# chenglou/ai-font-renderer

Measured on AMD Instinct MI355X. Metric: glyphs/sec training (batch fwd+bwd+step), higher is better.
Workload: dtype bf16; 1 GPU; C3: 32x32 glyph MLP 32->1024->1024->1024, char+font embedding, batch 8192/GPU (BASELINE configs[2]; per-GPU shard of configs[3]); per_gpu_batch=8192, global_batch=8192, parallelism=single, params=2137152

## Files before the change

ai-font-renderer_amd/csrc/afr_api.hip:

```cpp
#include "afr_common.h"
#include "../../include/afr.h"
static_assert(AFR_LOSS_MSE == LOSS_MSE && AFR_LOSS_BCE == LOSS_BCE, "afr.h and afr_common.h name the same loss kinds");

#include <cmath>
#include <cstdarg>
#include <cstdio>
#include <cstring>
#include <map>
#include <string>
#include <utility>
#include <vector>

static thread_local char g_err[512] = "";
static int fail(int code, const char* fmt, ...) {
    va_list ap;
    va_start(ap, fmt);
    vsnprintf(g_err, sizeof g_err, fmt, ap);
    va_end(ap);
    return code;
}
#define HIPCHK(expr)                                                                          \
    do {                                                                                      \
        hipError_t e_ = (expr);                                                               \
        if (e_ != hipSuccess) return fail(AFR_EHIP, "%s: %s", #expr, hipGetErrorString(e_)); \
// ... 2405 lines not shown
    if (tokens < 1) return fail(AFR_EINVAL, "afr_op_pixel_add_ln: tokens = %d must be >= 1", tokens);
    DevGuard dg(device_of(h));
    HIPCHK(afr_launch_pixel_add_ln(act_dtype, hin, h, pos, add, g, b, n, rows, tokens, d, eps, (hipStream_t)stream));
    return AFR_OK;
}
extern "C" int afr_op_pixel_attn(int act_dtype, const void* q, const void* kv, void* o, int64_t rows, int tokens, int d, int heads, int C,
                                 void* stream) {
    if (int rc = pixel_op_shape("afr_op_pixel_attn", act_dtype, rows, d)) return rc;
    if (int rc = pixel_op_attn_shape("afr_op_pixel_attn", tokens, d, heads, C)) return rc;
    if (!q || !kv || !o) return fail(AFR_EINVAL, "afr_op_pixel_attn: null argument");
    DevGuard dg(device_of(o));
    HIPCHK(afr_launch_pixel_attn(act_dtype, q, kv, o, rows, tokens, d, heads, C, (hipStream_t)stream));
    return AFR_OK;
}
extern "C" int afr_op_pixel_attn_bwd(int act_dtype, const void* dO, const void* q, const void* kv, void* dq, float* dkv_part, int B, int tokens,
                                     int d, int heads, int C, void* stream) {
    if (int rc = pixel_op_shape("afr_op_pixel_attn_bwd", act_dtype, B, d)) return rc;
    if (int rc = pixel_op_attn_shape("afr_op_pixel_attn_bwd", tokens, d, heads, C)) return rc;
    if (!dO || !q || !kv || !dq || !dkv_part) return fail(AFR_EINVAL, "afr_op_pixel_attn_bwd: null argument");
    const int chunk = afr_pixel_attn_chunk(tokens);
    if ((long long)B * ((tokens + chunk - 1) / chunk) >= (1ll << 31)) return fail(AFR_EUNSUPPORTED, "afr_op_pixel_attn_bwd: B * chunks must stay below 2^31");
    DevGuard dg(device_of(dq));
    HIPCHK(afr_launch_pixel_attn_bwd(act_dtype, dO, q, kv, dq, dkv_part, B, tokens, d, C, (hipStream_t)stream));
    return AFR_OK;
}
extern "C" int afr_op_pixel_head(int act_dtype, int loss_kind, const float* hin, float* h, const void* add, const float* g, const float* b,
                                 const float* w_out, const float* b_out, float* u, float* y, int64_t rows, int d, float eps, void* stream) {
    if (int rc = pixel_op_shape("afr_op_pixel_head", act_dtype, rows, d)) return rc;
    if (loss_kind != AFR_LOSS_MSE && loss_kind != AFR_LOSS_BCE) return fail(AFR_EINVAL, "afr_op_pixel_head: loss kind must be AFR_LOSS_MSE (0) or AFR_LOSS_BCE (1), got %d", loss_kind);
    if (!hin || !h || !add || !g || !b || !w_out || !b_out) return fail(AFR_EINVAL, "afr_op_pixel_head: null argument");
    DevGuard dg(device_of(h));
    HIPCHK(afr_launch_pixel_head(act_dtype, hin, h, add, g, b, w_out, b_out, u, y, rows, d, eps, (hipStream_t)stream, loss_kind));
    return AFR_OK;
}
extern "C" int afr_op_pixel_head_bwd(int act_dtype, const float* du, const float* hf, const float* g, const float* b, const float* w_out, float* dh,
                                     void* dhT, float* part, int64_t rows, int d, float eps, void* stream) {
    if (int rc = pixel_op_shape("afr_op_pixel_head_bwd", act_dtype, rows, d)) return rc;
    if (!du || !hf || !g || !b || !w_out || !dh || !part) return fail(AFR_EINVAL, "afr_op_pixel_head_bwd: null argument");
    DevGuard dg(device_of(dh));
    HIPCHK(afr_launch_pixel_head_bwd(act_dtype, du, hf, g, b, w_out, dh, dhT, part, rows, d, eps, (hipStream_t)stream));
    return AFR_OK;
}
extern "C" int afr_op_pixel_ln_bwd(int act_dtype, const void* dy, const float* hin, const float* g, float* dh, void* dhT, float* part, int64_t rows,
                                   int d, float eps, void* stream) {
    if (int rc = pixel_op_shape("afr_op_pixel_ln_bwd", act_dtype, rows, d)) return rc;
    if (!dy || !hin || !g || !dh || !part) return fail(AFR_EINVAL, "afr_op_pixel_ln_bwd: null argument");
    DevGuard dg(device_of(dh));
    HIPCHK(afr_launch_pixel_ln_bwd(act_dtype, dy, hin, g, dh, dhT, part, rows, d, eps, (hipStream_t)stream));
    return AFR_OK;
}

static int sheet_op_args(const char* what, int act_dtype, const afr_sheet_params* P, const int64_t* x, int ldx, int B, int L, int max_length,
                         int vocab, const afr_sheet_dropout* drop) {
    if (act_dtype != AFR_F32 && act_dtype != AFR_BF16) return fail(AFR_EINVAL, "%s: act_dtype must be AFR_F32 or AFR_BF16, got %d", what, act_dtype);
    if (B < 1) return fail(AFR_EINVAL, "%s: B = %d must be >= 1", what, B);
    if (L < 1) return fail(AFR_EINVAL, "%s: L = %d must be >= 1", what, L);
    if (max_length < 1 || vocab < 1) return fail(AFR_EINVAL, "%s: max_length = %d, vocab = %d must be >= 1", what, max_length, vocab);
    if (L > max_length) return fail(AFR_EINVAL, "%s: L = %d exceeds max_length = %d", what, L, max_length);
    if (L > 120) return fail(AFR_EUNSUPPORTED, "%s: L = %d exceeds 120 (a string's state must fit one compute unit's LDS)", what, L);
    if (ldx < L) return fail(AFR_EINVAL, "%s: ldx = %d is below L = %d", what, ldx, L);
    if ((long long)max_length * 32 >= (1ll << 31) || (long long)vocab * 32 >= (1ll << 31)) return fail(AFR_EUNSUPPORTED, "%s: a table must stay below 2^31 floats", what);
    if (!P || !x) return fail(AFR_EINVAL, "%s: null argument", what);
    if (!P->pos || !P->emb || !P->w_in || !P->b_in || !P->w_o || !P->b_o || !P->ln_g || !P->ln_b || !P->w1 || !P->b1)
        return fail(AFR_EINVAL, "%s: null parameter pointer", what);
    if (drop) {
        const float ps[3] = {drop->p_embed, drop->p_attn, drop->p_fc};
        for (float pr : ps)
            if (!(pr >= 0.f && pr < 1.f)) return fail(AFR_EINVAL, "%s: dropout rate %g outside [0, 1)", what, (double)pr);
    }
    return AFR_OK;
}
static SheetParams sheet_op_params(const afr_sheet_params* P) {
    SheetParams sp;
    sp.pos = P->pos; sp.emb = P->emb; sp.w_in = P->w_in; sp.b_in = P->b_in; sp.w_o = P->w_o; sp.b_o = P->b_o;
    sp.ln_g = P->ln_g; sp.ln_b = P->ln_b; sp.w1 = P->w1; sp.b1 = P->b1;
    return sp;
}
static SheetDrop sheet_op_drop(const afr_sheet_dropout* drop, float* save) {
    if (!drop) return sheet_drop(0, 0, 0, 0.f, 0.f, 0.f, 0, save);
    return sheet_drop(drop->seed, drop->step, drop->rank, drop->p_embed, drop->p_attn, drop->p_fc, 1, save);
}
extern "C" size_t afr_sheet_save_floats(int B, int L) {
    return B > 0 && L > 0 ? (size_t)B * (size_t)L * AFR_SHEET_SAVE_PER_POS : 0;
}
extern "C" int afr_op_sheet_fwd(int act_dtype, const afr_sheet_params* params, const int64_t* x, int ldx, int B, int L, int max_length, int vocab,
                                float ln_eps, const afr_sheet_dropout* drop, void* z, float* save, uint32_t* err, void* stream) {
    if (int rc = sheet_op_args("afr_op_sheet_fwd", act_dtype, params, x, ldx, B, L, max_length, vocab, drop)) return rc;
    if (!z) return fail(AFR_EINVAL, "afr_op_sheet_fwd: null argument");
    DevGuard dg(device_of(z));
    SheetDims d{L, max_length, 32, 4, 64, vocab};
    HIPCHK(afr_launch_sheet_fwd(act_dtype, d, sheet_op_params(params), sheet_op_drop(drop, save), x, ldx, B, z, ln_eps, err, (hipStream_t)stream));
    return AFR_OK;
}
extern "C" int afr_op_sheet_bwd(int act_dtype, const afr_sheet_params* params, const int64_t* x, int ldx, int B, int L, int max_length, int vocab,
                                float ln_eps, const afr_sheet_dropout* drop, const void* dz, const float* save, float* slabs,
                                const afr_sheet_slab_layout* lay, void* stream) {
    const char* what = "afr_op_sheet_bwd";
    if (int rc = sheet_op_args(what, act_dtype, params, x, ldx, B, L, max_length, vocab, drop)) return rc;
    if (!dz || !slabs || !lay) return fail(AFR_EINVAL, "%s: null argument", what);
    if (lay->total < 4 || (lay->total & 3)) return fail(AFR_EINVAL, "%s: total = %d must be a positive multiple of 4 (a block zeroes its slab 16 bytes at a time)", what, lay->total);
    if ((uintptr_t)slabs & 15) return fail(AFR_EINVAL, "%s: slabs must be 16-byte aligned", what);
    const long long off[10] = {lay->pos, lay->emb, lay->w_in, lay->b_in, lay->w_o, lay->b_o, lay->ln_g, lay->ln_b, lay->w1, lay->b1};
    const long long len[10] = {(long long)max_length * 32, (long long)vocab * 32, 96 * 32, 96, 32 * 32, 32, 32, 32, 64 * 32, 64};
    for (int i = 0; i < 10; ++i) {
        if (off[i] < 0 || off[i] + len[i] > lay->total) return fail(AFR_EINVAL, "%s: tensor %d (offset %lld, %lld floats) lies outside total = %d", what, i, off[i], len[i], lay->total);
        for (int j = 0; j < i; ++j)
            if (off[i] < off[j] + len[j] && off[j] < off[i] + len[i]) return fail(AFR_EINVAL, "%s: tensors %d and %d overlap", what, j, i);
    }
    DevGuard dg(device_of(slabs));
    SheetDims d{L, max_length, 32, 4, 64, vocab};
    SheetSlabOff so{lay->pos, lay->emb, lay->w_in, lay->b_in, lay->w_o, lay->b_o, lay->ln_g, lay->ln_b, lay->w1, lay->b1, lay->total};
    HIPCHK(afr_launch_sheet_bwd(act_dtype, d, sheet_op_params(params), sheet_op_drop(drop, const_cast<float*>(save)), x, ldx, B, dz, ln_eps, slabs, so,
                                (hipStream_t)stream));
    return AFR_OK;
}

constexpr size_t GLYPH_OP_LDS_MAX = 160 * 1024;
static int glyph_op_shape(const char* what, int act_dtype, int B, int E, int vocab, int n_fonts) {
    if (act_dtype != AFR_F32 && act_dtype != AFR_BF16) return fail(AFR_EINVAL, "%s: act_dtype must be AFR_F32 or AFR_BF16, got %d", what, act_dtype);
    if (B < 1) return fail(AFR_EINVAL, "%s: B = %d must be >= 1", what, B);
    if (vocab < 1 || n_fonts < 0) return fail(AFR_EINVAL, "%s: vocab = %d, n_fonts = %d", what, vocab, n_fonts);
    if (E < 8 || E % 8) return fail(AFR_EUNSUPPORTED, "%s: E = %d must be a positive multiple of 8", what, E);
    if ((long long)(vocab + (long long)n_fonts) * E >= (1ll << 31)) return fail(AFR_EUNSUPPORTED, "%s: a table must stay below 2^31 floats", what);
    return AFR_OK;
}
static int glyph_op_n1(const char* what, int N1) {
    if (N1 < 8 || N1 % 8) return fail(AFR_EUNSUPPORTED, "%s: N1 = %d must be a positive multiple of 8", what, N1);
    return AFR_OK;
}
static int glyph_op_fold(const char* what, int E, int vocab, int n_fonts) {
    const long long K0 = (long long)E + ((long long)vocab + n_fonts + 7) / 8 * 8;
    if (K0 > 512 || E > 128) return fail(AFR_EUNSUPPORTED, "%s: K0 = %lld, E = %d: the folded first layer takes K0 <= 512 and E <= 128", what, K0, E);
    return AFR_OK;
}
static int glyph_op_lds(const char* what, size_t lds) {
    if (lds > GLYPH_OP_LDS_MAX) return fail(AFR_EUNSUPPORTED, "%s: %zu bytes of dynamic LDS requested, above 160 KiB", what, lds);
    return AFR_OK;
}
extern "C" int afr_op_glyph_embed(int act_dtype, const float* emb, const float* femb, const int64_t* x, const int64_t* font, int B, int E, int vocab,
                                  int n_fonts, void* out, uint32_t* err, void* stream) {
    const char* what = "afr_op_glyph_embed";
    if (int rc = glyph_op_shape(what, act_dtype, B, E, vocab, n_fonts)) return rc;
    if (!emb || !x || !out || !err || (n_fonts > 0 && !femb)) return fail(AFR_EINVAL, "%s: null argument", what);
    DevGuard dg(device_of(out));
    HIPCHK(afr_launch_glyph_embed(act_dtype, emb, femb, x, font, B, E, vocab, n_fonts, out, err, (hipStream_t)stream));
    return AFR_OK;
}
extern "C" int afr_op_glyph_combo(const float* emb, const float* femb, const float* W1, const float* b1, const int64_t* x, const int64_t* font, int B,
                                  int E, int N1, int vocab, int n_fonts, void* h1c, int ld1, void* h0c, int32_t* cidx, void* w1t, uint32_t* err,
                                  void* stream) {
    const char* what = "afr_op_glyph_combo";
    if (int rc = glyph_op_shape(what, AFR_BF16, B, E, vocab, n_fonts)) return rc;
    if (int rc = glyph_op_n1(what, N1)) return rc;
    const size_t lds = (size_t)(256 * (E + 1) + 2 * 4 * E) * sizeof(float);
    if (lds > 48 * 1024) return fail(AFR_EUNSUPPORTED, "%s: E = %d needs %zu bytes of staging, above the kernel's 48 KiB (E <= 40)", what, E, lds);
    if (ld1 < N1) return fail(AFR_EINVAL, "%s: ld1 = %d is below N1 = %d", what, ld1, N1);
    if ((long long)vocab * (n_fonts > 0 ? n_fonts : 1) * (long long)ld1 >= (1ll << 31)) return fail(AFR_EUNSUPPORTED, "%s: the combination table must stay below 2^31 elements", what);
    if (!emb || !W1 || !b1 || !x || !h1c || !h0c || !cidx || !err || (n_fonts > 0 && !femb)) return fail(AFR_EINVAL, "%s: null argument", what);
    if ((uintptr_t)W1 & 15) return fail(AFR_EINVAL, "%s: W1 must be 16-byte aligned", what);
    DevGuard dg(device_of(h1c));
    HIPCHK(afr_launch_glyph_combo(emb, femb, W1, b1, x, font, B, E, N1, vocab, n_fonts, nullptr, h1c, ld1, h0c, cidx, err, (hipStream_t)stream, w1t));
    return AFR_OK;
}
extern "C" int afr_op_glyph_l1_bwd(const float* slabs, int nslabs, long long slab_stride, const float* W1, int N1, int E, int vocab, int n_fonts,
                                   float* dw1, float* dtab_part, void* stream) {
    const char* what = "afr_op_glyph_l1_bwd";
    if (int rc = glyph_op_shape(what, AFR_F32, 1, E, vocab, n_fonts)) return rc;
    if (int rc = glyph_op_n1(what, N1)) return rc;
    if (int rc = glyph_op_fold(what, E, vocab, n_fonts)) return rc;
    const int K0 = afr_glyph_k0(E, vocab, n_fonts);
    if (nslabs < 1) return fail(AFR_EINVAL, "%s: nslabs = %d must be >= 1", what, nslabs);
    if (slab_stride % 4 || (nslabs > 1 && slab_stride < (long long)N1 * K0))
        return fail(AFR_EINVAL, "%s: slab_stride = %lld must be a multiple of 4 and at least N1 * K0 = %lld", what, slab_stride, (long long)N1 * K0);
    if (!slabs || !W1 || !dw1 || !dtab_part) return fail(AFR_EINVAL, "%s: null argument", what);
    if ((uintptr_t)slabs & 15) return fail(AFR_EINVAL, "%s: slabs must be 16-byte aligned", what);
    const int G = std::max(1, std::min(1024 / (8 * K0 / 4), 8));
    if (int rc = glyph_op_lds(what, ((size_t)8 * (K0 + E) + (size_t)(G - 1) * 8 * K0) * sizeof(float))) return rc;
    DevGuard dg(device_of(dw1));
    HIPCHK(afr_launch_glyph_l1_bwd(slabs, nslabs, slab_stride, W1, N1, E, vocab, n_fonts, dw1, dtab_part, (hipStream_t)stream));
    return AFR_OK;
}
extern "C" int afr_op_glyph_l1_bwd_fused(const void* d1, const void* h0, int ldh, const int32_t* h0_rowmap, const void* W1T, const int64_t* x,
                                         const int64_t* font, int B, int N1, int vocab, int n_fonts, float* slabs, void* stream) {
    const char* what = "afr_op_glyph_l1_bwd_fused";
    if (int rc = glyph_op_shape(what, AFR_BF16, B, 32, vocab, n_fonts)) return rc;
    if (int rc = glyph_op_n1(what, N1)) return rc;
    if (!afr_glyph_l1_bwd_fused_eligible(AFR_BF16, 32, N1, vocab, n_fonts))
        return fail(AFR_EUNSUPPORTED, "%s: N1 = %d, vocab + n_fonts = %d: the fused backward takes N1 a multiple of 128 in 256 .. 1024 and at most 144 table rows (E = 32)",
                    what, N1, vocab + n_fonts);
    if (ldh < 32 || ldh % 8) return fail(AFR_EINVAL, "%s: ldh = %d must be a multiple of 8, at least 32", what, ldh);
    if ((long long)B * N1 * 2 >= (1ll << 31) || (!h0_rowmap && (long long)B * ldh * 2 >= (1ll << 31)))
        return fail(AFR_EUNSUPPORTED, "%s: d1 and h0 must stay below 2 GiB", what);
    if (!d1 || !h0 || !W1T || !x || !slabs) return fail(AFR_EINVAL, "%s: null argument", what);
    if (((uintptr_t)d1 & 15) || ((uintptr_t)h0 & 15) || ((uintptr_t)W1T & 15) || ((uintptr_t)slabs & 15))
        return fail(AFR_EINVAL, "%s: d1, h0, W1T and slabs must be 16-byte aligned", what);
    if (int rc = glyph_op_lds(what, (size_t)(N1 / afr_glyph_l1_bwd_fused_split(B, N1) / 128 + 1) * 16384 + 2 * 64 * sizeof(int))) return rc;
    DevGuard dg(device_of(slabs));
    HIPCHK(afr_launch_glyph_l1_bwd_fused(d1, N1, h0, ldh, W1T, x, font, B, N1, vocab, n_fonts, slabs, (hipStream_t)stream, h0_rowmap, nullptr));
    return AFR_OK;
}
extern "C" int afr_op_glyph_embed_bwd(int act_dtype, const void* d, const int64_t* x, const int64_t* font, int B, int E, int vocab, int n_fonts,
                                      float* slabs, void* stream) {
    const char* what = "afr_op_glyph_embed_bwd";
    if (int rc = glyph_op_shape(what, act_dtype, B, E, vocab, n_fonts)) return rc;
    if (int rc = glyph_op_lds(what, afr_glyph_embed_bwd_lds_bytes(E, vocab, n_fonts))) return rc;
    if (!d || !x || !slabs) return fail(AFR_EINVAL, "%s: null argument", what);
    DevGuard dg(device_of(slabs));
    HIPCHK(afr_launch_glyph_embed_bwd(act_dtype, d, x, font, B, E, vocab, n_fonts, slabs, (hipStream_t)stream));
    return AFR_OK;
}

extern "C" int afr_op_glyph_l1_fwd(int act_dtype, const float* emb, const float* femb, const float* W1, const float* b1, const int64_t* x,
                                   const int64_t* font, int B, int E, int N1, int vocab, int n_fonts, float* table, void* h0p, void* h1, void* w1t,
                                   uint32_t* err, void* stream) {
    const char* what = "afr_op_glyph_l1_fwd";
    if (int rc = glyph_op_shape(what, act_dtype, B, E, vocab, n_fonts)) return rc;
    if (int rc = glyph_op_n1(what, N1)) return rc;
    if (int rc = glyph_op_fold(what, E, vocab, n_fonts)) return rc;
    if ((long long)B * std::max(N1, afr_glyph_k0(E, vocab, n_fonts)) >= (1ll << 31) || (long long)(vocab + n_fonts) * N1 >= (1ll << 31))
        return fail(AFR_EUNSUPPORTED, "%s: h1, h0' and the table must stay below 2^31 elements", what);
    if (!emb || !W1 || !b1 || !x || !table || !h0p || !h1 || !err || (n_fonts > 0 && !femb)) return fail(AFR_EINVAL, "%s: null argument", what);
    if (((uintptr_t)emb & 15) || (n_fonts > 0 && ((uintptr_t)femb & 15)) ||((uintptr_t)W1 & 15) || ((uintptr_t)b1 & 15) || ((uintptr_t)table & 15) ||
        ((uintptr_t)h0p & 15) || ((uintptr_t)h1 & 15))
        return fail(AFR_EINVAL, "%s: emb, femb, W1, b1, table, h0p and h1 must be 16-byte aligned", what);
    DevGuard dg(device_of(h1));
    HIPCHK(afr_launch_glyph_l1_fwd(act_dtype, emb, femb, W1, b1, x, font, B, E, N1, vocab, n_fonts, table, h0p, h1, err, (hipStream_t)stream, w1t));
    return AFR_OK;
}
extern "C" int afr_glyph1_blocks(int dtype, int B, int P) {
    const int R = afr_glyph1_rows(dtype);
    return B < 1 ? 0 : (B + R - 1) / R * afr_glyph1_colsplit(dtype, B, P);
}
extern "C" int afr_op_glyph1_step(int dtype, int loss_kind, const float* emb, const float* femb, const void* W1, const float* b1, const void* W2,
                                  const float* b2, const void* W1T, const void* W2T, const int64_t* x, const int64_t* font, const void* target,
                                  int target_dtype, const int32_t* target_rows, int B, int E, int N1, int P, int vocab, int n_fonts,
                                  int64_t mean_elems, float* slabs, const afr_glyph1_layout* lay, float* loss_accum, float* loss_scratch,
                                  uint32_t* err, void* stream) {
    const char* what = "afr_op_glyph1_step";
    if (dtype != AFR_F32 && dtype != AFR_BF16) return fail(AFR_EINVAL, "%s: dtype must be AFR_F32 or AFR_BF16, got %d", what, dtype);
    if (loss_kind != AFR_LOSS_MSE && loss_kind != AFR_LOSS_BCE) return fail(AFR_EINVAL, "%s: loss kind must be AFR_LOSS_MSE (0) or AFR_LOSS_BCE (1), got %d", what, loss_kind);
    if (target_dtype != AFR_TARGET_U8 && target_dtype != AFR_TARGET_F32) return fail(AFR_EINVAL, "%s: target_dtype must be AFR_TARGET_U8 or AFR_TARGET_F32, got %d", what, target_dtype);
    if (B < 1) return fail(AFR_EINVAL, "%s: B = %d must be >= 1", what, B);
    if (vocab < 1 || n_fonts < 0) return fail(AFR_EINVAL, "%s: vocab = %d, n_fonts = %d", what, vocab, n_fonts);
    if (E < 1 || N1 < 1 || P < 1) return fail(AFR_EINVAL, "%s: E = %d, N1 = %d, P = %d must be >= 1", what, E, N1, P);
    if (mean_elems < 1) return fail(AFR_EINVAL, "%s: mean_elems = %lld must be >= 1", what, (long long)mean_elems);
    if (!afr_glyph1_eligible(E, N1, P, vocab, n_fonts))
        return fail(AFR_EUNSUPPORTED, "%s: E = %d, N1 = %d, P = %d, vocab + n_fonts = %d: the fused step takes E 32 or 64, N1 and P multiples of 64 up to 256 and at most 264 table rows",
                    what, E, N1, P, vocab + n_fonts);
    if (int rc = glyph_op_lds(what, afr_glyph1_lds_bytes(dtype, E, N1, P, vocab + n_fonts))) return rc;
    const bool b16 = dtype == AFR_BF16;
    if (!emb || !W1 || !b1 || !W2 || !b2 || !x || !target || !slabs || !lay || !loss_accum || !loss_scratch || !err || (n_fonts > 0 && !femb) ||
        (b16 && (!W1T || !W2T)))
        return fail(AFR_EINVAL, "%s: null argument", what);
    if (((uintptr_t)W1 & 15) || ((uintptr_t)W2 & 15) || (b16 && (((uintptr_t)W1T & 15) || ((uintptr_t)W2T & 15))) || ((uintptr_t)slabs & 15))
        return fail(AFR_EINVAL, "%s: W1, W2, W1T, W2T and slabs must be 16-byte aligned", what);
    if (lay->total < 4 || (lay->total & 3)) return fail(AFR_EINVAL, "%s: total = %d must be a positive multiple of 4", what, lay->total);
    const long long off[6] = {lay->emb, lay->font, lay->w1, lay->b1, lay->w2, lay->b2};
    const long long len[6] = {(long long)vocab * E, (long long)n_fonts * E, (long long)N1 * E, N1, (long long)P * N1, P};
    for (int i = 0; i < 6; ++i) {
        if (len[i] == 0) continue;
        if (off[i] < 0 || (off[i] & 3) || off[i] + len[i] > lay->total)
            return fail(AFR_EINVAL, "%s: tensor %d (offset %lld, %lld floats) must start on a multiple of 4 and lie inside total = %d", what, i, off[i], len[i], lay->total);
        for (int j = 0; j < i; ++j)
            if (len[j] && off[i] < off[j] + len[j] && off[j] < off[i] + len[i]) return fail(AFR_EINVAL, "%s: tensors %d and %d overlap", what, j, i);
    }
    DevGuard dg(device_of(slabs));
    Glyph1Args a;
    a.x = x; a.font = font;
    a.loss = loss_args(loss_scratch, true, loss_kind, target, target_dtype, target_rows, mean_elems, loss_accum);
    a.B = B; a.E = E; a.N1 = N1; a.P = P; a.vocab = vocab; a.n_fonts = n_fonts;
    a.emb = emb; a.femb = n_fonts > 0 ? femb : nullptr; a.b1 = b1; a.b2 = b2;
    a.W1 = W1; a.W2 = W2;
    a.W1T = b16 ? W1T : W1; a.W2T = b16 ? W2T : W2;
    a.slabs = slabs; a.slab_stride = lay->total;
    a.o_emb = lay->emb; a.o_font = n_fonts > 0 ? lay->font : 0; a.o_w1 = lay->w1; a.o_b1 = lay->b1; a.o_w2 = lay->w2; a.o_b2 = lay->b2;
    a.err = err;
    a.cs = afr_glyph1_colsplit(dtype, B, P);
    HIPCHK(afr_launch_glyph1_step(dtype, a, (hipStream_t)stream));
    return AFR_OK;
}
extern "C" int afr_op_transpose_bf16(const float* W, void* WT, int N, int K, void* stream) {
    const char* what = "afr_op_transpose_bf16";
    if (N < 1 || K < 1) return fail(AFR_EINVAL, "%s: N = %d, K = %d must be >= 1", what, N, K);
    if (!W || !WT) return fail(AFR_EINVAL, "%s: null argument", what);
    DevGuard dg(device_of(WT));
    HIPCHK(afr_launch_transpose_bf16(W, (bf16_t*)WT, N, K, (hipStream_t)stream));
    return AFR_OK;
}
```

ai-font-renderer_amd/csrc/elementwise.hip:

```cpp
#include <algorithm>
#include "afr_common.h"
#include "../../include/afr.h"

int afr_glyph_k0(int E, int vocab, int n_fonts);
static inline int grid_for(long long work_items, int block, int max_blocks = 2048) {
    long long g = (work_items + block - 1) / block;
    if (g < 1) g = 1;
    if (g > max_blocks) g = max_blocks;
    return (int)g;
}

__global__ __launch_bounds__(256) void reduce_slabs_kernel(float* __restrict__ dst, const float* __restrict__ slabs,
                                                           int nslabs, long long stride, long long n, float scale,
                                                           int accumulate) {
    const long long n4 = n >> 2;
    for (long long i = blockIdx.x * 256ll + threadIdx.x; i < n4; i += (long long)gridDim.x * 256) {
        float4 a = make_float4(0.f, 0.f, 0.f, 0.f);
        for (int s = 0; s < nslabs; ++s) {
            const float4 v = *reinterpret_cast<const float4*>(slabs + s * stride + 4 * i);
            a.x += v.x; a.y += v.y; a.z += v.z; a.w += v.w;
        }
        a.x *= scale; a.y *= scale; a.z *= scale; a.w *= scale;
        float4* d = reinterpret_cast<float4*>(dst) + i;
        if (accumulate) { float4 o = *d; a.x += o.x; a.y += o.y; a.z += o.z; a.w += o.w; }
// ... 820 lines not shown
        const int b = (int)(i / E), c = (int)(i % E);
        long long xi = x[b];
        if (xi < 0 || xi >= vocab) { if (c == 0) atomicOr(err_flag, 1u); xi = min(max(xi, 0ll), (long long)vocab - 1); }
        float v = emb[xi * E + c];
        if (n_fonts > 0) {
            long long fi = font ? font[b] : 0;
            if (fi < 0 || fi >= n_fonts) { if (c == 0) atomicOr(err_flag, 1u); fi = min(max(fi, 0ll), (long long)n_fonts - 1); }
            v += femb[fi * E + c];
        }
        out[i] = (T)v;
    }
}
hipError_t afr_launch_glyph_embed(int act_dtype, const float* emb, const float* font_emb, const int64_t* x,
                                  const int64_t* font, int B, int E, int vocab, int n_fonts, void* out,
                                  uint32_t* err_flag, hipStream_t s) {
    if (B <= 0) return hipSuccess;
    dim3 g(grid_for((long long)B * E, 256)), b(256);
    if (act_dtype == AFR_BF16)
        hipLaunchKernelGGL(glyph_embed_kernel<bf16_t>, g, b, 0, s, emb, font_emb, x, font, B, E, vocab, n_fonts, (bf16_t*)out, err_flag);
    else
        hipLaunchKernelGGL(glyph_embed_kernel<float>, g, b, 0, s, emb, font_emb, x, font, B, E, vocab, n_fonts, (float*)out, err_flag);
    return hipGetLastError();
}

constexpr int GT_ROWS = 2;
__global__ __launch_bounds__(256) void glyph_table_kernel(const float* __restrict__ emb, const float* __restrict__ femb,
                                                          const float* __restrict__ W1, int vocab, int rows, int E, int N1,
                                                          float* __restrict__ table, bf16_t* __restrict__ w1t) {
    extern __shared__ float sm[];
    float* Ws = sm;
    float* tab = sm + 256 * (E + 1);
    const int r0 = blockIdx.x * GT_ROWS, n0 = blockIdx.y * 256;
    const int nn = min(256, N1 - n0), nr = min(GT_ROWS, rows - r0);
    const int E4 = E >> 2;
    for (int i = threadIdx.x; i < nn * E4; i += 256) {
        const float4 v = *reinterpret_cast<const float4*>(W1 + (size_t)n0 * E + 4 * i);
        float* d = Ws + (i / E4) * (E + 1) + 4 * (i % E4);
        d[0] = v.x; d[1] = v.y; d[2] = v.z; d[3] = v.w;
    }
    for (int i = threadIdx.x; i < nr * E; i += 256) {
        const int r = r0 + i / E, k = i % E;
        tab[i] = r < vocab ? emb[(size_t)r * E + k] : femb[(size_t)(r - vocab) * E + k];
    }
    __syncthreads();
    if ((int)threadIdx.x >= nn) return;
    const float* w = Ws + threadIdx.x * (E + 1);
    if (w1t && blockIdx.x == 0)
        for (int k = 0; k < E; ++k) w1t[(size_t)k * N1 + n0 + threadIdx.x] = (bf16_t)w[k];
    float a[GT_ROWS];
#pragma unroll
    for (int j = 0; j < GT_ROWS; ++j) a[j] = 0.f;
    for (int k = 0; k < E; ++k) {
        const float wv = w[k];
#pragma unroll
        for (int j = 0; j < GT_ROWS; ++j) a[j] = fmaf(tab[j * E + k], wv, a[j]);
    }
    for (int j = 0; j < nr; ++j) table[(size_t)(r0 + j) * N1 + n0 + threadIdx.x] = a[j];
}
template <typename T>
__device__ __forceinline__ void store8(T* q, const float (&v)[8]) {
    if constexpr (sizeof(T) == 2) {
        bf16x8 w;
#pragma unroll
        for (int r = 0; r < 8; ++r) w[r] = (bf16_t)v[r];
        __builtin_nontemporal_store(w, reinterpret_cast<bf16x8*>(q));
    } else {
        const f32x4 lo = {v[0], v[1], v[2], v[3]}, hi = {v[4], v[5], v[6], v[7]};
        __builtin_nontemporal_store(lo, reinterpret_cast<f32x4*>(q));
        __builtin_nontemporal_store(hi, reinterpret_cast<f32x4*>(q) + 1);
    }
}
template <typename T>
__global__ __launch_bounds__(256) void glyph_l1_fwd_kernel(const float* __restrict__ table, const float* __restrict__ b1,
                                                           const float* __restrict__ emb, const float* __restrict__ femb,
                                                           const int64_t* __restrict__ x, const int64_t* __restrict__ font,
                                                           int B, int E, int N1, int vocab, int n_fonts, int K0,
                                                           T* __restrict__ h0, T* __restrict__ h1, uint32_t* err_flag) {
    const int c1 = N1 >> 3, c0 = K0 >> 3;
    const int b = blockIdx.x * blockDim.y + threadIdx.y;
    if (b >= B) return;
    long long xi = x[b];
    if (xi < 0 || xi >= vocab) { if (threadIdx.x == 0) atomicOr(err_flag, 1u); xi = min(max(xi, 0ll), (long long)vocab - 1); }
    long long fi = 0;
    if (n_fonts > 0) {
        fi = font ? font[b] : 0;
        if (fi < 0 || fi >= n_fonts) { if (threadIdx.x == 0) atomicOr(err_flag, 1u); fi = min(max(fi, 0ll), (long long)n_fonts - 1); }
    }
    const float* trow_c = table + (size_t)xi * N1;
    const float* trow_f = table + (size_t)(vocab + fi) * N1;
    for (int c = threadIdx.x; c < c1; c += blockDim.x) {
        float v[8];
        const int n = 8 * c;
        const float4 a0 = *reinterpret_cast<const float4*>(trow_c + n), a1 = *reinterpret_cast<const float4*>(trow_c + n + 4);
        const float4 g0 = *reinterpret_cast<const float4*>(b1 + n), g1 = *reinterpret_cast<const float4*>(b1 + n + 4);
        v[0] = a0.x + g0.x; v[1] = a0.y + g0.y; v[2] = a0.z + g0.z; v[3] = a0.w + g0.w;
        v[4] = a1.x + g1.x; v[5] = a1.y + g1.y; v[6] = a1.z + g1.z; v[7] = a1.w + g1.w;
        if (n_fonts > 0) {
            const float4 f0 = *reinterpret_cast<const float4*>(trow_f + n), f1 = *reinterpret_cast<const float4*>(trow_f + n + 4);
            v[0] += f0.x; v[1] += f0.y; v[2] += f0.z; v[3] += f0.w; v[4] += f1.x; v[5] += f1.y; v[6] += f1.z; v[7] += f1.w;
        }
#pragma unroll
        for (int r = 0; r < 8; ++r) v[r] = fmaxf(v[r], 0.f);
        store8(h1 + (size_t)b * N1 + n, v);
    }
    for (int c = threadIdx.x; c < c0; c += blockDim.x) {
        float v[8];
        const int k0 = 8 * c;
        if (k0 < E) {
            const float* e = emb + (size_t)xi * E + k0;
            const float4 a0 = *reinterpret_cast<const float4*>(e), a1 = *reinterpret_cast<const float4*>(e + 4);
            v[0] = a0.x; v[1] = a0.y; v[2] = a0.z; v[3] = a0.w; v[4] = a1.x; v[5] = a1.y; v[6] = a1.z; v[7] = a1.w;
            if (n_fonts > 0) {
                const float* f = femb + (size_t)fi * E + k0;
                const float4 f0 = *reinterpret_cast<const float4*>(f), f1 = *reinterpret_cast<const float4*>(f + 4);
                v[0] += f0.x; v[1] += f0.y; v[2] += f0.z; v[3] += f0.w; v[4] += f1.x; v[5] += f1.y; v[6] += f1.z; v[7] += f1.w;
            }
        } else {
            const int r0 = k0 - E, hx = (int)xi, hf = n_fonts > 0 ? vocab + (int)fi : -1;
#pragma unroll
            for (int r = 0; r < 8; ++r) v[r] = (r0 + r == hx || r0 + r == hf) ? 1.f : 0.f;
        }
        store8(h0 + (size_t)b * K0 + k0, v);
    }
}
hipError_t afr_launch_glyph_l1_fwd(int act_dtype, const float* emb, const float* font_emb, const float* W1, const float* b1,
                                   const int64_t* x, const int64_t* font, int B, int E, int N1, int vocab, int n_fonts,
                                   float* table, void* h0, void* h1, uint32_t* err_flag, hipStream_t s, void* w1t) {
    if (B <= 0) return hipSuccess;
    if ((N1 & 7) || (E & 7)) return hipErrorInvalidValue;
    const int K0 = afr_glyph_k0(E, vocab, n_fonts);
    const int rows = vocab + n_fonts;
    const size_t tlds = (size_t)(256 * (E + 1) + GT_ROWS * E) * sizeof(float);
    static size_t tlds_set[16];
    int dev = 0;
    if (tlds > 48 * 1024 && hipGetDevice(&dev) == hipSuccess && (dev < 0 || dev >= 16 || tlds_set[dev] < tlds)) {
        hipError_t e = hipFuncSetAttribute((const void*)glyph_table_kernel, hipFuncAttributeMaxDynamicSharedMemorySize, (int)tlds);
        if (e != hipSuccess) return e;
        if (dev >= 0 && dev < 16) tlds_set[dev] = tlds;
    }
    hipLaunchKernelGGL(glyph_table_kernel, dim3((rows + GT_ROWS - 1) / GT_ROWS, (N1 + 255) / 256), dim3(256), tlds, s, emb, font_emb,
                       W1, vocab, rows, E, N1, table, (bf16_t*)w1t);
    int tx = 32;
    while (tx < 128 && tx < N1 / 8) tx *= 2;
    dim3 b(tx, 256 / tx), g((B + b.y - 1) / b.y);
    if (act_dtype == AFR_BF16)
        hipLaunchKernelGGL(glyph_l1_fwd_kernel<bf16_t>, g, b, 0, s, table, b1, emb, font_emb, x, font, B, E, N1, vocab, n_fonts, K0,
                           (bf16_t*)h0, (bf16_t*)h1, err_flag);
    else
        hipLaunchKernelGGL(glyph_l1_fwd_kernel<float>, g, b, 0, s, table, b1, emb, font_emb, x, font, B, E, N1, vocab, n_fonts, K0,
                           (float*)h0, (float*)h1, err_flag);
    return hipGetLastError();
}

constexpr int CB_COMBOS = 4;
__global__ __launch_bounds__(256) void glyph_combo_kernel(const float* __restrict__ W1, const float* __restrict__ b1,
                                                          const float* __restrict__ emb, const float* __restrict__ femb,
                                                          const int64_t* __restrict__ x, const int64_t* __restrict__ font,
                                                          int B, int E, int N1, int vocab, int n_fonts, int combo_blocks,
                                                          bf16_t* __restrict__ h1c, int ld1, bf16_t* __restrict__ h0c, int* __restrict__ cidx,
                                                          bf16_t* __restrict__ w1t, uint32_t* err_flag) {
    extern __shared__ float sm[];
    const int nf = max(n_fonts, 1), ncombo = vocab * nf;
    if ((int)blockIdx.x >= combo_blocks) {
        if (blockIdx.y != 0) return;
        const int b = ((int)blockIdx.x - combo_blocks) * 256 + threadIdx.x;
        if (b >= B) return;
        long long xi = x[b], fi = (n_fonts > 0 && font) ? font[b] : 0;
        if (xi < 0 || xi >= vocab) { atomicOr(err_flag, 1u); xi = min(max(xi, 0ll), (long long)vocab - 1); }
        if (n_fonts > 0 && (fi < 0 || fi >= n_fonts)) { atomicOr(err_flag, 1u); fi = min(max(fi, 0ll), (long long)n_fonts - 1); }
        cidx[b] = (int)(xi * nf + fi);
        return;
    }
    float* Ws = sm;
    float* er = sm + 256 * (E + 1);
    float* fr = er + CB_COMBOS * E;
    const int c0 = blockIdx.x * CB_COMBOS, n0 = blockIdx.y * 256;
    const int nn = min(256, N1 - n0), nc = min(CB_COMBOS, ncombo - c0);
    const int E4 = E >> 2;
    for (int i = threadIdx.x; i < nn * E4; i += 256) {
        const float4 v = *reinterpret_cast<const float4*>(W1 + (size_t)n0 * E + 4 * i);
        float* d = Ws + (i / E4) * (E + 1) + 4 * (i % E4);
        d[0] = v.x; d[1] = v.y; d[2] = v.z; d[3] = v.w;
    }
    for (int i = threadIdx.x; i < nc * E; i += 256) {
        const int c = c0 + i / E, k = i % E, xi = c / nf, fi = c - xi * nf;
        er[i] = emb[(size_t)xi * E + k];
        fr[i] = n_fonts > 0 ? femb[(size_t)fi * E + k] : 0.f;
        if (blockIdx.y == 0) h0c[(size_t)c * E + k] = (bf16_t)(n_fonts > 0 ? er[i] + fr[i] : er[i]);
    }
    __syncthreads();
    if ((int)threadIdx.x >= nn) return;
    const float* w = Ws + threadIdx.x * (E + 1);
    if (w1t && blockIdx.x == 0)
        for (int k = 0; k < E; ++k) w1t[(size_t)k * N1 + n0 + threadIdx.x] = (bf16_t)w[k];
    float tc[CB_COMBOS], tf[CB_COMBOS];
#pragma unroll
    for (int j = 0; j < CB_COMBOS; ++j) tc[j] = tf[j] = 0.f;
    for (int k = 0; k < E; ++k) {
        const float wv = w[k];
#pragma unroll
        for (int j = 0; j < CB_COMBOS; ++j) {
            tc[j] = fmaf(er[j * E + k], wv, tc[j]);
            tf[j] = fmaf(fr[j * E + k], wv, tf[j]);
        }
    }
    const float bias = b1[n0 + threadIdx.x];
    for (int j = 0; j < nc; ++j) {
        float v = tc[j] + bias;
        if (n_fonts > 0) v += tf[j];
        h1c[(size_t)(c0 + j) * ld1 + n0 + threadIdx.x] = (bf16_t)fmaxf(v, 0.f);
    }
}
hipError_t afr_launch_glyph_combo(const float* emb, const float* font_emb, const float* W1, const float* b1, const int64_t* x,
                                  const int64_t* font, int B, int E, int N1, int vocab, int n_fonts, float* table, void* h1c,
                                  int ld1, void* h0c, int* cidx, uint32_t* err_flag, hipStream_t s, void* w1t) {
    if (B <= 0) return hipSuccess;
    if ((N1 & 7) || (E & 7) || E > 256) return hipErrorInvalidValue;
    (void)table;
    const size_t lds = (size_t)(256 * (E + 1) + 2 * CB_COMBOS * E) * sizeof(float);
    if (lds > 48 * 1024) return hipErrorInvalidValue;
    const int ncombo = vocab * (n_fonts > 0 ? n_fonts : 1);
    const int combo_blocks = (ncombo + CB_COMBOS - 1) / CB_COMBOS;
    hipLaunchKernelGGL(glyph_combo_kernel, dim3(combo_blocks + (B + 255) / 256, (N1 + 255) / 256), dim3(256), lds, s, W1, b1, emb, font_emb,
                       x, font, B, E, N1, vocab, n_fonts, combo_blocks, (bf16_t*)h1c, ld1, (bf16_t*)h0c, cidx, (bf16_t*)w1t, err_flag);
    return hipGetLastError();
}

int afr_glyph_k0(int E, int vocab, int n_fonts) { return E + (vocab + n_fonts + 7) / 8 * 8; }

constexpr int GL1_ROWS = 8, GL1_NT = 1024;
__global__ __launch_bounds__(GL1_NT) void glyph_l1_bwd_kernel(const float* __restrict__ slabs, int nslabs, long long slab_stride,
                                                              const float* __restrict__ W1, int N1, int E, int R, int K0,
                                                              float* __restrict__ dw1, float* __restrict__ dtab_part) {
    extern __shared__ float sm[];
    float* S = sm;
    float* W = sm + GL1_ROWS * K0;
    float* part = W + GL1_ROWS * E;
    const int n0 = blockIdx.x * GL1_ROWS;
    const int nr = min(GL1_ROWS, N1 - n0);
    const int cnt4 = nr * K0 / 4;
    const int full4 = GL1_ROWS * K0 / 4;
    const int G = max(1, min(GL1_NT / full4, 8));
    const int g = threadIdx.x / full4, i = threadIdx.x % full4;
    if (g < G && i < cnt4) {
        const float* src = slabs + (size_t)n0 * K0 + 4 * i;
        float4 a = make_float4(0.f, 0.f, 0.f, 0.f);
#pragma unroll 4
        for (int z = g; z < nslabs; z += G) {
            const float4 v = *reinterpret_cast<const float4*>(src + (long long)z * slab_stride);
            a.x += v.x; a.y += v.y; a.z += v.z; a.w += v.w;
        }
        float* dst = g == 0 ? S : part + (size_t)(g - 1) * GL1_ROWS * K0;
        *reinterpret_cast<float4*>(dst + 4 * i) = a;
    }
    for (int j = threadIdx.x; j < nr * E; j += GL1_NT) W[j] = W1[(size_t)n0 * E + j];
    __syncthreads();
    if ((int)threadIdx.x < cnt4) {
        float4 a = *reinterpret_cast<float4*>(S + 4 * threadIdx.x);
        for (int q = 1; q < G; ++q) {
            const float4 v = *reinterpret_cast<const float4*>(part + (size_t)(q - 1) * GL1_ROWS * K0 + 4 * threadIdx.x);
            a.x += v.x; a.y += v.y; a.z += v.z; a.w += v.w;
        }
        *reinterpret_cast<float4*>(S + 4 * threadIdx.x) = a;
    }
    __syncthreads();
    for (int j = threadIdx.x; j < nr * E; j += GL1_NT) dw1[(size_t)n0 * E + j] = S[(j / E) * K0 + (j % E)];
    float* out = dtab_part + (size_t)blockIdx.x * R * E;
    for (int j = threadIdx.x; j < R * E; j += GL1_NT) {
        const int r = j / E, k = j % E;
        float a = 0.f;
        for (int q = 0; q < nr; ++q) a = fmaf(S[q * K0 + E + r], W[q * E + k], a);
        out[j] = a;
    }
}
int afr_glyph_l1_bwd_blocks(int N1) { return (N1 + GL1_ROWS - 1) / GL1_ROWS; }
hipError_t afr_launch_glyph_l1_bwd(const float* slabs, int nslabs, long long slab_stride, const float* W1, int N1, int E,
                                   int vocab, int n_fonts, float* dw1, float* dtab_part, hipStream_t s) {
    const int K0 = afr_glyph_k0(E, vocab, n_fonts);
    if (GL1_ROWS * K0 / 4 > GL1_NT) return hipErrorInvalidValue;
    const int G = std::max(1, std::min(GL1_NT / (GL1_ROWS * K0 / 4), 8));
    const size_t lds = ((size_t)GL1_ROWS * (K0 + E) + (size_t)(G - 1) * GL1_ROWS * K0) * sizeof(float);
    hipLaunchKernelGGL(glyph_l1_bwd_kernel, dim3(afr_glyph_l1_bwd_blocks(N1)), dim3(GL1_NT), lds, s, slabs, nslabs, slab_stride, W1, N1,
                       E, vocab + n_fonts, K0, dw1, dtab_part);
    return hipGetLastError();
}

constexpr int EMB_BWD_ROWS = 32;
template <typename T>
__global__ __launch_bounds__(256) void glyph_embed_bwd_kernel(const T* __restrict__ d, const int64_t* __restrict__ x,
                                                              const int64_t* __restrict__ font, int B, int E, int vocab,
                                                              int n_fonts, float* __restrict__ slabs) {
    extern __shared__ float sm[];
    const int rows_tot = vocab + n_fonts;
    const int LDT = E + 1;
    float* acc = sm;
    float* tile = sm + (size_t)rows_tot * E;
    int* ids = reinterpret_cast<int*>(tile + (size_t)EMB_BWD_ROWS * LDT);
    int* fids = ids + EMB_BWD_ROWS;
    const int b0 = blockIdx.x * EMB_BWD_ROWS;
    const int nb = min(EMB_BWD_ROWS, B - b0);
    for (int i = threadIdx.x; i < rows_tot * E; i += 256) acc[i] = 0.f;
    for (int i = threadIdx.x; i < nb * E; i += 256) tile[(i / E) * LDT + (i % E)] = (float)d[(size_t)b0 * E + i];
    if ((int)threadIdx.x < nb) {
        long long xi = x[b0 + threadIdx.x];
        ids[threadIdx.x] = (int)min(max(xi, 0ll), (long long)vocab - 1);
        long long fi = (n_fonts > 0 && font) ? font[b0 + threadIdx.x] : 0;
        fids[threadIdx.x] = (int)min(max(fi, 0ll), (long long)max(n_fonts, 1) - 1);
    }
    __syncthreads();
    const int slot = threadIdx.x >> 5, c0 = threadIdx.x & 31;
    for (int c = c0; c < E; c += 32) {
        for (int r = 0; r < nb; ++r) {
            const int v = ids[r];
            const float val = tile[r * LDT + c];
            if ((v & 7) == slot) acc[v * E + c] += val;
            if (n_fonts > 0) {
                const int f = fids[r];
                if ((f & 7) == slot) acc[(vocab + f) * E + c] += val;
            }
        }
    }
    __syncthreads();
    float* out = slabs + (size_t)blockIdx.x * rows_tot * E;
    for (int i = threadIdx.x; i < rows_tot * E; i += 256) out[i] = acc[i];
}
int afr_embed_bwd_blocks(int B) { return (B + EMB_BWD_ROWS - 1) / EMB_BWD_ROWS; }
size_t afr_glyph_embed_bwd_lds_bytes(int E, int vocab, int n_fonts) {
    return ((size_t)(vocab + n_fonts) * E + (size_t)EMB_BWD_ROWS * (E + 1)) * sizeof(float) + 2 * EMB_BWD_ROWS * sizeof(int);
}
hipError_t afr_launch_glyph_embed_bwd(int act_dtype, const void* d, const int64_t* x, const int64_t* font, int B, int E,
                                      int vocab, int n_fonts, float* slabs, hipStream_t s) {
    if (B <= 0) return hipSuccess;
    const size_t lds = afr_glyph_embed_bwd_lds_bytes(E, vocab, n_fonts);
    if (lds > 160 * 1024) return hipErrorInvalidValue;
    static size_t set[2][16];
    int dev = 0;
    const int ti = act_dtype == AFR_BF16 ? 1 : 0;
    if (lds > 48 * 1024 && hipGetDevice(&dev) == hipSuccess && (dev < 0 || dev >= 16 || set[ti][dev] < lds)) {
        hipError_t e = ti ? hipFuncSetAttribute((const void*)glyph_embed_bwd_kernel<bf16_t>, hipFuncAttributeMaxDynamicSharedMemorySize, (int)lds)
                          : hipFuncSetAttribute((const void*)glyph_embed_bwd_kernel<float>, hipFuncAttributeMaxDynamicSharedMemorySize, (int)lds);
        if (e != hipSuccess) return e;
        if (dev >= 0 && dev < 16) set[ti][dev] = lds;
    }
    dim3 g(afr_embed_bwd_blocks(B)), b(256);
    if (act_dtype == AFR_BF16)
        hipLaunchKernelGGL(glyph_embed_bwd_kernel<bf16_t>, g, b, lds, s, (const bf16_t*)d, x, font, B, E, vocab, n_fonts, slabs);
    else
        hipLaunchKernelGGL(glyph_embed_bwd_kernel<float>, g, b, lds, s, (const float*)d, x, font, B, E, vocab, n_fonts, slabs);
    return hipGetLastError();
}
```

Measured before the change: 46.23 million glyphs/s.

## Rewrite glyph combo kernel to keep W1 rows in registers instead of LDS

The combination-table forward kernel no longer stages 256 W1 rows and embeddings in LDS. Each thread now holds one W1 row in registers as float4s, and each wave handles 4 combos (16 per block) over 64-row chunks, reading embeddings straight from global/cache. It is templated on E=32 and on whether fonts are present, so the loops unroll fully and the font branches compile away. The change drops LDS use and the block barrier and launches more, smaller blocks, in exchange for repeated global embedding reads and E now capped at 40.

```diff
diff --git a/ai-font-renderer_amd/csrc/afr_api.hip b/ai-font-renderer_amd/csrc/afr_api.hip
--- a/ai-font-renderer_amd/csrc/afr_api.hip
+++ b/ai-font-renderer_amd/csrc/afr_api.hip
@@ -2581,8 +2581,7 @@
     const char* what = "afr_op_glyph_combo";
     if (int rc = glyph_op_shape(what, AFR_BF16, B, E, vocab, n_fonts)) return rc;
     if (int rc = glyph_op_n1(what, N1)) return rc;
-    const size_t lds = (size_t)(256 * (E + 1) + 2 * 4 * E) * sizeof(float);
-    if (lds > 48 * 1024) return fail(AFR_EUNSUPPORTED, "%s: E = %d needs %zu bytes of staging, above the kernel's 48 KiB (E <= 40)", what, E, lds);
+    if (E > 40) return fail(AFR_EUNSUPPORTED, "%s: E = %d is above the kernel's E <= 40 (a W1 row per thread; formerly 48 KiB of staging)", what, E);
     if (ld1 < N1) return fail(AFR_EINVAL, "%s: ld1 = %d is below N1 = %d", what, ld1, N1);
     if ((long long)vocab * (n_fonts > 0 ? n_fonts : 1) * (long long)ld1 >= (1ll << 31)) return fail(AFR_EUNSUPPORTED, "%s: the combination table must stay below 2^31 elements", what);
     if (!emb || !W1 || !b1 || !x || !h1c || !h0c || !cidx || !err || (n_fonts > 0 && !femb)) return fail(AFR_EINVAL, "%s: null argument", what);
diff --git a/ai-font-renderer_amd/csrc/elementwise.hip b/ai-font-renderer_amd/csrc/elementwise.hip
--- a/ai-font-renderer_amd/csrc/elementwise.hip
+++ b/ai-font-renderer_amd/csrc/elementwise.hip
@@ -996,18 +996,20 @@
     return hipGetLastError();
 }
 
-constexpr int CB_COMBOS = 4;
+constexpr int CB_COMBOS = 16, CB_ROWS = 64, CB_PER = 4, CB_MAXE = 40;
+template <int EC, bool FONTS>
 __global__ __launch_bounds__(256) void glyph_combo_kernel(const float* __restrict__ W1, const float* __restrict__ b1,
                                                           const float* __restrict__ emb, const float* __restrict__ femb,
                                                           const int64_t* __restrict__ x, const int64_t* __restrict__ font,
-                                                          int B, int E, int N1, int vocab, int n_fonts, int combo_blocks,
+                                                          int B, int E_, int N1, int vocab, int n_fonts, int combo_blocks,
                                                           bf16_t* __restrict__ h1c, int ld1, bf16_t* __restrict__ h0c, int* __restrict__ cidx,
                                                           bf16_t* __restrict__ w1t, uint32_t* err_flag) {
-    extern __shared__ float sm[];
+    const int E = EC ? EC : E_;
+    constexpr int KQ = (EC ? EC : CB_MAXE) / 4;
     const int nf = max(n_fonts, 1), ncombo = vocab * nf;
-    if ((int)blockIdx.x >= combo_blocks) {
-        if (blockIdx.y != 0) return;
-        const int b = ((int)blockIdx.x - combo_blocks) * 256 + threadIdx.x;
+    const int row_chunks = (N1 + CB_ROWS - 1) / CB_ROWS;
+    if ((int)blockIdx.x >= combo_blocks * row_chunks) {
+        const int b = ((int)blockIdx.x - combo_blocks * row_chunks) * 256 + threadIdx.x;
         if (b >= B) return;
         long long xi = x[b], fi = (n_fonts > 0 && font) ? font[b] : 0;
         if (xi < 0 || xi >= vocab) { atomicOr(err_flag, 1u); xi = min(max(xi, 0ll), (long long)vocab - 1); }
@@ -1015,44 +1017,62 @@
         cidx[b] = (int)(xi * nf + fi);
         return;
     }
-    float* Ws = sm;
-    float* er = sm + 256 * (E + 1);
-    float* fr = er + CB_COMBOS * E;
-    const int c0 = blockIdx.x * CB_COMBOS, n0 = blockIdx.y * 256;
-    const int nn = min(256, N1 - n0), nc = min(CB_COMBOS, ncombo - c0);
-    const int E4 = E >> 2;
-    for (int i = threadIdx.x; i < nn * E4; i += 256) {
-        const float4 v = *reinterpret_cast<const float4*>(W1 + (size_t)n0 * E + 4 * i);
-        float* d = Ws + (i / E4) * (E + 1) + 4 * (i % E4);
-        d[0] = v.x; d[1] = v.y; d[2] = v.z; d[3] = v.w;
-    }
-    for (int i = threadIdx.x; i < nc * E; i += 256) {
-        const int c = c0 + i / E, k = i % E, xi = c / nf, fi = c - xi * nf;
-        er[i] = emb[(size_t)xi * E + k];
-        fr[i] = n_fonts > 0 ? femb[(size_t)fi * E + k] : 0.f;
-        if (blockIdx.y == 0) h0c[(size_t)c * E + k] = (bf16_t)(n_fonts > 0 ? er[i] + fr[i] : er[i]);
-    }
-    __syncthreads();
-    if ((int)threadIdx.x >= nn) return;
-    const float* w = Ws + threadIdx.x * (E + 1);
-    if (w1t && blockIdx.x == 0)
-        for (int k = 0; k < E; ++k) w1t[(size_t)k * N1 + n0 + threadIdx.x] = (bf16_t)w[k];
-    float tc[CB_COMBOS], tf[CB_COMBOS];
-#pragma unroll
-    for (int j = 0; j < CB_COMBOS; ++j) tc[j] = tf[j] = 0.f;
-    for (int k = 0; k < E; ++k) {
-        const float wv = w[k];
-#pragma unroll
-        for (int j = 0; j < CB_COMBOS; ++j) {
-            tc[j] = fmaf(er[j * E + k], wv, tc[j]);
-            tf[j] = fmaf(fr[j * E + k], wv, tf[j]);
-        }
-    }
-    const float bias = b1[n0 + threadIdx.x];
-    for (int j = 0; j < nc; ++j) {
-        float v = tc[j] + bias;
-        if (n_fonts > 0) v += tf[j];
-        h1c[(size_t)(c0 + j) * ld1 + n0 + threadIdx.x] = (bf16_t)fmaxf(v, 0.f);
+    const int cb = blockIdx.x / row_chunks, rc = blockIdx.x - cb * row_chunks;
+    const int wave = __builtin_amdgcn_readfirstlane(threadIdx.x >> 6);
+    const int n = rc * CB_ROWS + (threadIdx.x & 63), c0 = cb * CB_COMBOS;
+    const bool row = n < N1;
+    float4 w[KQ];
+#pragma unroll
+    for (int kk = 0; kk < KQ; ++kk)
+        w[kk] = (4 * kk < E && row) ? *reinterpret_cast<const float4*>(W1 + (size_t)n * E + 4 * kk) : make_float4(0.f, 0.f, 0.f, 0.f);
+    const float bias = row ? b1[n] : 0.f;
+    if (rc == 0)
+        for (int i = threadIdx.x; i < min(CB_COMBOS, ncombo - c0) * E; i += 256) {
+            const int c = c0 + i / E, k = i % E, xi = c / nf, fi = c - xi * nf;
+            const float e = emb[(size_t)xi * E + k];
+            h0c[(size_t)c * E + k] = (bf16_t)(FONTS ? e + femb[(size_t)fi * E + k] : e);
+        }
+    if (w1t && cb == 0 && row) {
+#pragma unroll
+        for (int kk = 0; kk < KQ; ++kk)
+            if (4 * kk < E && (kk & 3) == wave) {
+                bf16_t* d = w1t + (size_t)(4 * kk) * N1 + n;
+                d[0] = (bf16_t)w[kk].x; d[N1] = (bf16_t)w[kk].y; d[2 * (size_t)N1] = (bf16_t)w[kk].z; d[3 * (size_t)N1] = (bf16_t)w[kk].w;
+            }
+    }
+    const int cw = c0 + wave * CB_PER;
+    float tc[CB_PER], tf[CB_PER];
+#pragma unroll
+    for (int j = 0; j < CB_PER; ++j) {
+        const int c = min(cw + j, ncombo - 1), xi = c / nf, fi = c - xi * nf;
+        const float* er = emb + (size_t)xi * E;
+        const float* fr = FONTS ? femb + (size_t)fi * E : er;
+        tc[j] = tf[j] = 0.f;
+#pragma unroll
+        for (int kk = 0; kk < KQ; ++kk) {
+            if (4 * kk < E) {
+                const float wk[4] = {w[kk].x, w[kk].y, w[kk].z, w[kk].w};
+                const float4 e4 = *reinterpret_cast<const float4*>(er + 4 * kk);
+                const float ev[4] = {e4.x, e4.y, e4.z, e4.w};
+#pragma unroll
+                for (int u = 0; u < 4; ++u) tc[j] = fmaf(ev[u], wk[u], tc[j]);
+                if (FONTS) {
+                    const float4 f4 = *reinterpret_cast<const float4*>(fr + 4 * kk);
+                    const float fv[4] = {f4.x, f4.y, f4.z, f4.w};
+#pragma unroll
+                    for (int u = 0; u < 4; ++u) tf[j] = fmaf(fv[u], wk[u], tf[j]);
+                }
+            }
+        }
+    }
+    if (!row) return;
+#pragma unroll
+    for (int j = 0; j < CB_PER; ++j) {
+        if (cw + j < ncombo) {
+            float v = tc[j] + bias;
+            if (FONTS) v += tf[j];
+            h1c[(size_t)(cw + j) * ld1 + n] = (bf16_t)fmaxf(v, 0.f);
+        }
     }
 }
 hipError_t afr_launch_glyph_combo(const float* emb, const float* font_emb, const float* W1, const float* b1, const int64_t* x,
@@ -1061,12 +1081,16 @@
     if (B <= 0) return hipSuccess;
     if ((N1 & 7) || (E & 7) || E > 256) return hipErrorInvalidValue;
     (void)table;
-    const size_t lds = (size_t)(256 * (E + 1) + 2 * CB_COMBOS * E) * sizeof(float);
-    if (lds > 48 * 1024) return hipErrorInvalidValue;
+    if (E > CB_MAXE) return hipErrorInvalidValue;
     const int ncombo = vocab * (n_fonts > 0 ? n_fonts : 1);
     const int combo_blocks = (ncombo + CB_COMBOS - 1) / CB_COMBOS;
-    hipLaunchKernelGGL(glyph_combo_kernel, dim3(combo_blocks + (B + 255) / 256, (N1 + 255) / 256), dim3(256), lds, s, W1, b1, emb, font_emb,
-                       x, font, B, E, N1, vocab, n_fonts, combo_blocks, (bf16_t*)h1c, ld1, (bf16_t*)h0c, cidx, (bf16_t*)w1t, err_flag);
+    const dim3 grid(combo_blocks * ((N1 + CB_ROWS - 1) / CB_ROWS) + (B + 255) / 256);
+    auto launch = [&](auto kernel) {
+        hipLaunchKernelGGL(kernel, grid, dim3(256), 0, s, W1, b1, emb, font_emb, x, font, B, E, N1, vocab, n_fonts, combo_blocks, (bf16_t*)h1c, ld1,
+                           (bf16_t*)h0c, cidx, (bf16_t*)w1t, err_flag);
+    };
+    if (E == 32) n_fonts > 0 ? launch(glyph_combo_kernel<32, true>) : launch(glyph_combo_kernel<32, false>);
+    else n_fonts > 0 ? launch(glyph_combo_kernel<0, true>) : launch(glyph_combo_kernel<0, false>);
     return hipGetLastError();
 }
 
```

Result: faster. 47.15 million glyphs/s (median of 6 runs) (+2.0%).
